# doing-science-to-stuff/ndt

Hardware: AMD Instinct MI355X
Metric: Mray/s (primary+shadow+reflect) at 1920x1080 (higher is better)
Workload: dtype f64

## Files before the change

### ndt_amd/csrc/ndt_device.hpp

```cpp
#pragma once
#include <hip/hip_runtime.h>
#include <stdint.h>

#define NDT_EPS   (1e-4)
#define NDT_EPS2  ((NDT_EPS) * (NDT_EPS))
#define NDT_INV_EPS2 (1.0 / (NDT_EPS2))
#define NDT_DBL_MAX 1.7976931348623157e308
#define NDT_PI 3.14159265358979323846

#define NDT_DEV __device__ __forceinline__

#define NDT_F_TYPE_MASK   0xff
#define NDT_F_GATE        0x100
#define NDT_F_INF_ENDS    0x200
#define NDT_F_USE_NORMALS 0x400
#define NDT_F_TRANSPARENT 0x800
#define NDT_F_BOX         0x1000
#define NDT_F_FACEBOX     0x2000
#define NDT_F_OBOX        0x4000
#define NDT_F_FACETREE    0x8000
#define NDT_F_FACEGROUPS  0x10000

enum { T_SPHERE = 0, T_HPLANE, T_HDISK, T_CYLINDER, T_HCYLINDER, T_ORTHOTOPE, T_HCUBE, T_HFACET, T_FACET };
enum { NDT_LIGHT_AMBIENT_ = 0, NDT_LIGHT_POINT_ = 1, NDT_LIGHT_DIRECTIONAL_ = 2, NDT_LIGHT_SPOT_ = 3 };
// ... 1211 lines not shown
            record_of(__ffsll((long long)any) - 1, flags, words, m, at, sph);
            const double t0 = word_of(lane, words, at, sph), t1 = word_of(lane + 64, words, at, sph);
            put(l_par, flags, words, m, t0, t1);
            cls_lds_sync();
        }
        while (any != 0ull) {
            const int k = __ffsll((long long)any) - 1;
            any &= any - 1ull;
            int n_flags = 0, n_words = 0, n_m = 0, n_at = 0, n_sph = 0;
            double t0 = 0.0, t1 = 0.0;
            if (any != 0ull) {
                record_of(__ffsll((long long)any) - 1, n_flags, n_words, n_m, n_at, n_sph);
                t0 = word_of(lane, n_words, n_at, n_sph);
                t1 = word_of(lane + 64, n_words, n_at, n_sph);
            }
            const long long rbits = __double_as_longlong(l_ref[k]);
            const int id = __builtin_amdgcn_readfirstlane((int)(rbits & 0xffffffffll));
            const int flags = __builtin_amdgcn_readfirstlane((int)(rbits >> 32));
            const double *rec = l_par + cur * par_stride;
            bool pass = open != 0 && ((want >> k) & 1ull);
            if ((flags & NDT_F_GATE) && pass) pass = bsphere_gate<N>(rec, sd_par, 0, o, v, min_dist);
            if (pass) {
                double res[N], nrm[N];
                if (isect<N, false>(rec, sd_par, 0, o, v, res, nrm)) {
                    const double dist = v_dist<N>(o, res);
                    if (dist > NDT_EPS && (dist + NDT_EPS < min_dist || min_dist < 0)) {
                        min_dist = dist;
                        best = id;
                    }
                    if (dist_limit == 0.0 || dist < dist_limit) {
                        open = 0;
                        last = id;
                    }
                }
            }
            cur ^= 1;
            if (any != 0ull) put(l_par + cur * par_stride, n_flags, n_words, n_m, t0, t1);
            cls_lds_sync();
            if (__ballot(open != 0) == 0ull) any = 0ull;
        }
        cls_lds_sync();
        NDT_STAMP(2);
        if (open) last = (int)(__double_as_longlong(l_ref[cnt - 1]) & 0xffffffffll);
        cls_lds_sync();
    }
}

#define NDT_KD_STACK 40
#define NDT_STACK_FLAG 0x40000000



struct KdStackLds {
    double *tu;
    int *node;
    int stride;
};

template <int N, int MW, bool LSTACK = false, bool UNI = false, bool LAZY_INV = false>
NDT_DEV void trace_kd(const double *blob, const SceneDesc &sd, VisitMask<MW> &mask, const double (&o)[N],
                      const double (&v)[N], double dist_limit, int &out_obj, int &out_prim
#ifdef NDT_PHASE_TIMING
                      , unsigned long long (&ph)[8], unsigned int (&cnt)[8], unsigned int (&occ)[8]
#endif
                      , KdStackLds ls = KdStackLds{}, ClsLds cl = ClsLds{}, const bool has_ray = true, double *box_slot = nullptr)
{
#ifdef NDT_PHASE_TIMING
    unsigned long long ph_last = __builtin_readcyclecounter();
#endif
#ifdef NDT_T1_KEEP_INV
    constexpr bool KEEP_INV = true;
#else
    constexpr bool KEEP_INV = (MW != 0);
#endif
    auto inv_of = [](double v_i) {
        double r;
        if (v_i < NDT_EPS2 && v_i >= 0.0)
            r = NDT_INV_EPS2;
        else if (v_i > -NDT_EPS2 && v_i <= 0.0)
            r = -NDT_INV_EPS2;
        else
            r = 1.0 / v_i;
        return r;
    };
    double v_inv[N];
    if (KEEP_INV && !LAZY_INV) {
#pragma unroll
        for (int i = 0; i < N; ++i) v_inv[i] = inv_of(v[i]);
    }
    auto inv_at = [&](int dim) {
        if constexpr (KEEP_INV) return v_pick<N>(v_inv, dim);
        else return inv_of(v_pick<N>(v, dim));
    };
    NDT_STAMP(5);

    double t_inf = NDT_DBL_MAX;
    int inf_obj = -1, inf_prim = -1;
    double lt = NDT_DBL_MAX;
    int l_obj = -1, l_prim = -1;

    int st_node[LSTACK ? 1 : NDT_KD_STACK];
    double st_a[LSTACK ? 1 : NDT_KD_STACK], st_tu[LSTACK ? 1 : NDT_KD_STACK];
    int sp = 0;
    int node = 0;
    double ntl = 0, ntu = 0;
    int st = 4;
    bool boxed = false;

    constexpr bool BITS = (MW == 1);
    unsigned long long cand = 0ull;
    int sec = 0, pos = 0, end = 0;
    double min_dist = -1;
    int best_obj = -1, best_prim = -1;
    int sub_i = 0, sub_end = 0, sub_owner = -1, sub_prim = -1;
    long long sub_live = -1;
    double sub_min = -1;

    if (!has_ray) {
        st = 3;
    } else if (sd.n_inf > 0) {
        st = 5;
        if (BITS) {
            cand = sd.inf_bits;
        } else {
            sec = sd.off_inf;
            pos = 0;
            end = sd.n_inf;
        }
    }

    while (true) {
        if (st == 4) {
            double tl = -NDT_DBL_MAX, tu = NDT_DBL_MAX;
            bool box = true;
#pragma unroll
            for (int i = 0; i < N; ++i) {
                if (box) {
                    double v_i = v[i], o_i = o[i];
                    if (!(fabs(v_i) < NDT_EPS2)) {
                        double tl_i = (blob[sd.off_bb + i] - o_i) / v_i;
                        double tu_i = (blob[sd.off_bb + N + i] - o_i) / v_i;
                        if (tl_i > tu_i) {
                            double tmp = tl_i;
                            tl_i = tu_i;
                            tu_i = tmp;
                        }
                        if (tl_i > tl) tl = tl_i;
                        if (tu_i < tu) tu = tu_i;
                        if (tu < -NDT_EPS) box = false;
                    }
                }
            }
            if (box) {
                tl -= NDT_EPS;
                tu += NDT_EPS;
                box = (tu >= -NDT_EPS) && (tl <= tu);
            }
            if (!box || sd.n_kd_nodes <= 0) {
                st = 3;
            } else {
                mask.clear(sd.mask_words);
                if (BITS && sd.gate_bits != 0ull) {
                    unsigned long long todo = sd.gate_bits, dead = 0ull;
                    while (todo != 0ull) {
                        const int id = __ffsll((long long)todo) - 1;
                        todo &= todo - 1ull;
                        const int b = sd.off_bs + id * (N + 2);
                        double c[N], oc[N];
                        blob_vec<N>(blob, b, c);
                        v_sub<N>(o, c, oc);
                        const double oc_len2 = v_dot<N>(oc, oc);
                        const double voc = v_dot<N>(v, oc);
                        const double voc2 = voc * voc;
                        const double desc = voc2 - oc_len2 + blob[b + N + 1];
                        if (desc < 0.0 || (voc > 0.0 && voc2 > desc)) dead |= 1ull << id;
                    }
                    mask.w[0] |= dead;
                }
                if (KEEP_INV && LAZY_INV) {
#pragma unroll
                    for (int i = 0; i < N; ++i) {
                        double v_i = v[i];
                        asm volatile("" : "+v"(v_i));
                        v_inv[i] = inv_of(v_i);
                    }
                }
                node = 0;
                ntl = tl;
                ntu = tu;
                st = 1;
            }
        }
        {
            while (st < 2) {
                NDT_OCC(0);
                if (st == 0) {
                    if (sp == 0) {
                        st = 3;
                    } else {
                        sp -= LSTACK ? ls.stride : 1;
                        double a;
                        if (LSTACK) {
                            const int parent = ls.node[sp];
                            ntu = ls.tu[sp];
                            const ndt_v2d prec = blob_pair(blob, sd.off_kd + 2 * parent);
                            const long long pw0 = __double_as_longlong(prec.x);
                            const int pdim = (int)(pw0 & 0xffffffffll);
                            const double pv_inv = inv_at(pdim);
                            a = (prec.y - v_pick<N>(o, pdim)) * pv_inv;
                            node = (pv_inv < NDT_EPS2) ? parent + 1 : (int)(pw0 >> 32);
                        } else {
                            node = st_node[sp];
                            a = st_a[sp];
                            ntu = st_tu[sp];
                        }
                        ntl = a - NDT_EPS;
                        st = ((lt > a) & !(ntu < 0.0)) ? 1 : 0;
                    }
                } else if (ntu < 0.0) {
                    st = 0;
                }
                if (st == 1) {
                    NDT_COUNT(0);
                    ndt_v2d rec = blob_pair(blob, sd.off_kd + 2 * node);
                    unsigned long long below = ~0ull;
                    if (BITS) {
                        double ns = blob[sd.off_nset + node];
#ifndef NDT_NO_T_HOIST
                        asm volatile("" : "+v"(rec.x), "+v"(rec.y), "+v"(ns));
#endif
                        below = (unsigned long long)__double_as_longlong(ns) & ~mask.w[0];
                    }
                    const long long w0 = __double_as_longlong(rec.x);
                    const int dim = (int)(w0 & 0xffffffffll);
                    if (BITS && below == 0ull) {
                        st = 0;
                    } else if (dim < 0) {
                        if (BITS) {
                            st = 2;
                            cand = below;
                        } else {
                            const long long w1 = __double_as_longlong(rec.y);
                            const int num = (int)(w1 >> 32);
                            st = num > 0 ? 2 : 0;
                            sec = sd.off_leaf;
                            pos = (int)(w1 & 0xffffffffll);
                            end = pos + num;
                        }
                    } else {
                        const double boundary = rec.y;
                        const double v_inv_i = inv_at(dim);
                        const double o_i = v_pick<N>(o, dim);
                        const bool swap = v_inv_i < NDT_EPS2;
                        const int left = node + 1, right = (int)(w0 >> 32);
                        const int near = swap ? right : left, far = swap ? left : right;
                        const double tp = (boundary - o_i) * v_inv_i;
                        const bool alive = lt > ntl;
                        const bool near_only = (ntu < tp - NDT_EPS) & alive;
                        const bool far_only = !near_only & (ntl > tp + NDT_EPS) & alive;
                        const bool both = !near_only & !far_only;
                        if (both & (lt > tp)) {
                            if (LSTACK) { ls.node[sp] = node; ls.tu[sp] = ntu; }
                            else { st_node[sp] = far; st_a[sp] = tp; st_tu[sp] = ntu; }
                            sp += LSTACK ? ls.stride : 1;
                        }
                        const bool go_near = near_only | (both & alive);
                        ntu = (both & alive) ? tp + NDT_EPS : ntu;
                        node = go_near ? near : far;
                        st = (go_near | far_only) ? 1 : 0;
                    }
                }
            }
        }
        NDT_STAMP(0);
        const bool have_list = st == 2 || st == 5, list_is_inf = st == 5;
        if (UNI ? (__ballot(have_list) == 0ull) : !have_list) break;

        min_dist = -1;
        best_obj = -1;
        best_prim = -1;
        bool list_open = have_list;
        bool scanned_together = false;
        if (UNI && MW == 0 && cl.base) {
            const bool elig = have_list && !list_is_inf && mask.hist_n >= 0;
            unsigned long long todo = __ballot(elig);
            const int n_listed = __popcll(__ballot(have_list));
            while (todo != 0ull) {
                const int leader = __ffsll((long long)todo) - 1;
                const int w0 = __builtin_amdgcn_readlane(sec + pos, leader), e0 = __builtin_amdgcn_readlane(sec + end, leader);
                bool mine = elig && sec + pos == w0;
                const unsigned long long group = __ballot(mine);
                todo &= ~group;
                if (__popcll(group) < cl.min_group && !(__popcll(group) == n_listed && n_listed >= 16)) mine = false;
                if (__ballot(mine) == 0ull) continue;
                double md;
                int best, last;
                NDT_STAMP(3);
#ifdef NDT_PHASE_TIMING
                cls_scan<N, MW>(blob, sd, mask, cl.base, mine, o, v, dist_limit, w0, e0, box_slot, boxed, md, best, last, ph, ph_last);
#else
                cls_scan<N, MW>(blob, sd, mask, cl.base, mine, o, v, dist_limit, w0, e0, box_slot, boxed, md, best, last);
#endif
                if (mine) {
                    min_dist = md;
                    best_obj = best;
                    best_prim = best;
                    mask.end_leaf(blob_int(blob, sd.off_kd + 2 * node, 1), last);
                    list_open = false;
                    scanned_together = true;
                }
            }
        }
        int gs = list_open ? 0 : 4;
        while (gs != 4) {
            int prim = -1;
// ... 218 lines not shown
```

### ndt_amd/csrc/ndt_kernels.hip

```cpp
#if NDT_DIMS <= 5 && !defined(NDT_OUTLINE_SMALL)
#define NDT_INLINE_LIBM 1
#endif
#if NDT_DIMS <= 7 && !defined(NDT_OUTLINE_SMALL)
#define NDT_SHADE_INLINE_ISECT 1
#endif
#include "ndt_kernels.hpp"
#include "ndt_shading.hpp"
#include <hip/hip_ext.h>
#include <stdlib.h>
#include <map>
#include <mutex>
#include <tuple>

#ifndef NDT_DIMS
#error "compile with -DNDT_DIMS=<3..10>"
#endif
#define NDT_CAT2(a, b) a##b
#define NDT_CAT(a, b) NDT_CAT2(a, b)

namespace NDT_CAT(ndt_d, NDT_DIMS) {

static constexpr int N = NDT_DIMS;


// ... 222 lines not shown
    mask.h0 = mask.h1 = mask.h2 = mask.h3 = 0u;
    mask.hist_n = -1;
    mask.slab_words = sd.mask_words;
    mask.ls.sets = nullptr;
    mask.ls.blob = gblob;
    mask.ls.words = sd.mask_words;
    mask.ls.off_lrange = sd.off_lrange;
    mask.ls.off_leaf = sd.off_leaf;
    mask.ls.cap = sd.hist_cap;
    if (MW == 0) {
        const long long lane_slot = (long long)blockIdx.x * blockDim.x + threadIdx.x;
        mask.ext = ws.mask_slab + lane_slot;
        mask.ext_stride = (int)ws.mask_slab_lanes;
        if (sd.off_lset > 0) mask.ls.sets = reinterpret_cast<const unsigned long long *>(gblob + sd.off_lset);
    }
}

NDT_DEV int seg_light_origin(const double *gblob, const SceneDesc &sd, int s)
{
    unsigned long long rest = ~sd.ambient_bits;
    for (int k = 0; k < s; ++k) rest &= rest - 1ull;
    const int li = __ffsll((long long)rest) - 1;
    const int w = sd.off_lights + li * (6 + 4 * N);
    const int type = blob_int(gblob, w, 0);
    return (type == NDT_LIGHT_POINT_ || type == NDT_LIGHT_SPOT_) ? w + 5 : -1;
}

typedef __attribute__((address_space(4))) const char *KernargBytes;
struct TraceKernargs {
    const double *gblob;
    SceneDesc sd;
    Workspace ws;
    TraceJob job;
};
constexpr size_t KARG_TRACE_WS = offsetof(TraceKernargs, ws);
constexpr size_t KARG_TRACE_JOB = offsetof(TraceKernargs, job);
#ifdef NDT_HEAD_STEPS
constexpr int trace_head_steps(int, int mw, bool, bool) { return mw != 0 ? (NDT_HEAD_STEPS) : 0; }
#else
constexpr int trace_head_steps(int n, int mw, bool lstack, bool prim)
{
    if (mw == 0) return 0;
    if (prim) return 7;
    if (n == 4 && mw == 4 && lstack) return 5;
    if (n == 4 && mw == 1 && !lstack) return 0;
    if (n == 5 && lstack) return 5;
    if (n == 6 && mw == 1 && !lstack) return 0;
    if (n == 8 && mw == 1 && !lstack) return 1;
    if (n == 10 && !lstack) return 5;
    if (n == 11 && !(mw == 1 && lstack)) return 0;
    return 7;
}
#endif
NDT_DEV KernargBytes karg_here()
{
    KernargBytes p = (KernargBytes)__builtin_amdgcn_kernarg_segment_ptr();
    asm volatile("" : "+s"(p));
    return p;
}
template <typename T> NDT_DEV T karg_get(KernargBytes p)
{
    static_assert(sizeof(T) % 4 == 0 && std::is_trivially_copyable<T>::value, "words");
    union { T v; unsigned int w[sizeof(T) / 4]; } u;
#pragma unroll
    for (size_t i = 0; i < sizeof(T) / 4; ++i) u.w[i] = reinterpret_cast<__attribute__((address_space(4))) const unsigned int *>(p)[i];
    return u.v;
}
#define NDT_KARG_PTR(obj, base, member) \
    (obj).member = *reinterpret_cast<__attribute__((address_space(4))) decltype((obj).member) const *>((base) + offsetof(decltype(obj), member))
NDT_DEV TracePart karg_trace_part(bool in_seg)
{
    const int at = in_seg ? (int)offsetof(TraceJob, seg) : (int)offsetof(TraceJob, dense);
    const KernargBytes kp = karg_here() + KARG_TRACE_JOB + __builtin_amdgcn_readfirstlane(at);
    TracePart p = karg_get<TracePart>(kp);
    NDT_KARG_PTR(p, kp, o); NDT_KARG_PTR(p, kp, v); NDT_KARG_PTR(p, kp, lim); NDT_KARG_PTR(p, kp, valid);
    NDT_KARG_PTR(p, kp, out_obj); NDT_KARG_PTR(p, kp, out_prim);
    return p;
}
NDT_DEV Workspace karg_trace_workspace(KernargBytes ka)
{
    const KernargBytes kp = ka + KARG_TRACE_WS;
    Workspace w = karg_get<Workspace>(kp);
    NDT_KARG_PTR(w, kp, ray_o); NDT_KARG_PTR(w, kp, ray_v); NDT_KARG_PTR(w, kp, frac); NDT_KARG_PTR(w, kp, depth_left);
    NDT_KARG_PTR(w, kp, hit_obj); NDT_KARG_PTR(w, kp, child_refl); NDT_KARG_PTR(w, kp, child_refr); NDT_KARG_PTR(w, kp, sh_mask);
    NDT_KARG_PTR(w, kp, count); NDT_KARG_PTR(w, kp, rng_key);
    return w;
}
NDT_DEV RenderGeom karg_trace_geom(KernargBytes ka)
{
    const KernargBytes kp = ka + KARG_TRACE_JOB + offsetof(TraceJob, rg);
    RenderGeom rg = karg_get<RenderGeom>(kp);
    NDT_KARG_PTR(rg, kp, samples); NDT_KARG_PTR(rg, kp, sample_keys);
    return rg;
}

#ifndef NDT_TICKET_AHEAD
#define NDT_TICKET_AHEAD 256
#endif
template <int MW, bool LDS, bool LSTACK = false, bool PRIM = false>
__global__ void __launch_bounds__(MW == 0 ? NDT_TRACE_T1_MAX_BLOCK : NDT_TRACE_MAX_BLOCK) k_trace(const double *__restrict__ gblob, SceneDesc sd, Workspace ws, TraceJob job)
{
    constexpr int STEPS = trace_head_steps(N, MW, LSTACK, PRIM);
    constexpr bool KARG = (STEPS & 1) != 0, SEG_ONCE = (STEPS & 2) != 0, LAZY = (STEPS & 4) != 0;
    extern __shared__ __attribute__((aligned(16))) double lds_blob[];
    const double *blob = gblob;
    if (LDS) {
        const int pairs = sd.trace_words >> 1;
        const ndt_v2d *src2 = reinterpret_cast<const ndt_v2d *>(gblob);
        ndt_v2d *dst2 = reinterpret_cast<ndt_v2d *>(lds_blob);
        int i = threadIdx.x;
        for (; i + 3 * (int)blockDim.x < pairs; i += 4 * blockDim.x) {
            const ndt_v2d a = src2[i], b = src2[i + blockDim.x], c = src2[i + 2 * blockDim.x], d = src2[i + 3 * blockDim.x];
            dst2[i] = a; dst2[i + blockDim.x] = b; dst2[i + 2 * blockDim.x] = c; dst2[i + 3 * blockDim.x] = d;
        }
        for (; i < pairs; i += blockDim.x) dst2[i] = src2[i];
        if ((sd.trace_words & 1) && threadIdx.x == 0) lds_blob[sd.trace_words - 1] = gblob[sd.trace_words - 1];
        __syncthreads();
        blob = lds_blob;
    }
    KdStackLds kstack{};
    if (LSTACK) {
        double *base = lds_blob + ((sd.trace_words + 1) & ~1);
        const int depth = sd.kd_depth + 1;
        kstack.stride = blockDim.x;
        kstack.tu = base + threadIdx.x;
        kstack.node = (int *)(base + (size_t)depth * blockDim.x) + threadIdx.x;
    }
    VisitMask<MW> mask;
    init_visit_mask<MW>(mask, gblob, sd, ws);
    ClsLds cls{};
    double *box_slot = nullptr;
    if (MW == 0 && !LDS) {
        const int wave = threadIdx.x >> 6, waves = blockDim.x >> 6;
        const int box_words = sd.off_obox > 0 ? N * 128 : 0;
        if (sd.off_obox > 0) box_slot = lds_blob + (size_t)wave * box_words + 2 * (threadIdx.x & 63);
        if (sd.cls_par_words > 0) {
            cls.base = lds_blob + (size_t)waves * box_words + (size_t)wave * cls_window_words<N>(sd.cls_par_words);
            cls.min_group = sd.cls_min_group;
        }
    }
    const int lane = __lane_id();
    const unsigned int probe_start = job.exit_log ? (unsigned int)wall_clock64() : 0u;
    unsigned int probe_batch = probe_start;
#ifdef NDT_PHASE_TIMING
    unsigned long long ph[8] = { 0, 0, 0, 0, 0, 0, 0, 0 };
    unsigned long long acc[24];
    for (int i = 0; i < 24; ++i) acc[i] = 0ull;
    unsigned long long out_last = __builtin_readcyclecounter();
    unsigned long long batch_mark = 0;
#endif
    const int bs = job.batch;
    const int sh = (bs == 64) ? 6 : (bs == 32) ? 5 : (bs == 16) ? 4 : 3;
    int seg_batches = 0, seg_batches_incl = 0, seg_cnt = 0;
    int seg_origin = -1;
    if (job.n_seg > 0) {
        seg_cnt = (lane < job.n_seg) ? job.seg_count[lane] : 0;
        const int excl = wave_excl_scan((seg_cnt + bs - 1) >> sh, seg_batches);
        seg_batches_incl = excl + ((seg_cnt + bs - 1) >> sh);
        if (SEG_ONCE && job.seg_light_origins && seg_cnt > 0) seg_origin = seg_light_origin(gblob, sd, lane);
    }
    long long dense_count = job.count, dense_begin = job.begin, seg_stride = job.seg_stride;
    if (job.levels) {
        const LevelRange cur = job.levels[job.seg_level];
        seg_stride = cur.seg_stride;
        LevelRange next;
        if (job.publish_level >= 0) {
            next.begin = cur.begin + cur.count;
            next.count = (long long)ws.counters[0] - next.begin;
            next.n_shadow = 0;
            if (next.count < 0 || (ws.counters[2] & 1) != 0) next.count = 0;
            next.seg_stride = (next.count + 63) & ~63LL;
            const bool sh_overflow = (long long)job.n_seg * next.seg_stride > ws.sh_cap;
            if (blockIdx.x == 0 && threadIdx.x < 64) {
                long long emitted = seg_cnt;
                for (int d = 32; d > 0; d >>= 1) emitted += __shfl_xor(emitted, d, 64);
                NDT_SEG_COUNTERS(ws, job.publish_level + 1)[lane] = 0;
                if (lane == 0) {
                    job_levels_mut(job)[job.publish_level].n_shadow = emitted;
                    LevelRange out = next;
                    if (sh_overflow) {
                        atomicOr(&ws.counters[2], 2);
                        const long long need = (long long)job.n_seg * next.seg_stride;
                        ws.counters[3] = need > 0x7fffffffLL ? 0x7fffffff : (int)need;
                        out.count = 0;
                        out.seg_stride = 0;
                    }
                    job_levels_mut(job)[job.publish_level + 1] = out;
                    ws.mail[job.publish_level + 1] = out;
                    __threadfence_system();
                    __hip_atomic_store(&ws.mail_tag[job.publish_level + 1], job.publish_tag, __ATOMIC_RELEASE, __HIP_MEMORY_SCOPE_SYSTEM);
                }
            }
            if (sh_overflow) next.count = 0;
        } else {
            next = job.levels[job.dense_level >= 0 ? job.dense_level : 0];
        }
        if (job.dense_level >= 0) {
            dense_begin = next.begin;
            dense_count = next.count;
// ... 66 lines not shown
            const int sb = (int)(b - dense_batches);
            const int s = __popcll(__ballot(lane < job.n_seg && seg_batches_incl <= sb));
            if (SEG_ONCE) origin_word = __builtin_amdgcn_readlane(seg_origin, __builtin_amdgcn_readfirstlane(s));
            else if (MW != 0 && job.seg_light_origins) origin_word = seg_light_origin(gblob, sd, __builtin_amdgcn_readfirstlane(s));
            const int first = (s > 0) ? __shfl(seg_batches_incl, s - 1, 64) : 0;
            const int cnt = __shfl(seg_cnt, s, 64);
            const int idx = (sb - first) * bs + lane;
            live = lane < bs && idx < cnt;
            g = (long long)s * seg_stride + (live ? idx : 0);
        } else {
            const long long r = b * bs + lane;
            live = lane < bs && r < dense_count;
            g = dense_begin + (live ? r : 0);
            if constexpr (KARG) {
                if (!PRIM && live) {
                    const int *valid = karg_trace_part(false).valid;
                    if (valid && valid[g] <= 0) live = false;
                }
            } else {
                if (!PRIM && live && job.dense.valid && job.dense.valid[g] <= 0) live = false;
            }
        }
        double o[N], v[N];
        const bool make = PRIM && !in_seg;
        if (PRIM && make && live) {
            if (KARG) {
                const KernargBytes ka = karg_here();
                live = primary_node<false, true>(gblob, sd, karg_trace_workspace(ka), karg_trace_geom(ka), g, o, v);
            } else {
                live = primary_node<false, true>(gblob, sd, ws, job.rg, g, o, v);
            }
        }
        if (live || MW == 0) {
        const TracePart part_here = KARG ? karg_trace_part(in_seg) : TracePart{};
        const TracePart &part = KARG ? part_here : in_seg ? job.seg : job.dense;
#ifdef NDT_TRACE_SKIP_KNOB
        if (job.skip_trace == 3) {
            for (int c = 0; c < N; ++c) { o[c] = (double)g; v[c] = 1.0; }
        } else
#endif
        if (live) {
            if (!make) {
                if (origin_word >= 0) blob_vec<N>(gblob, origin_word, o);
                else load_soa<N>(part.o, part.stride, g, o);
                load_soa<N>(part.v, part.stride, g, v);
            }
        } else {
#pragma unroll
            for (int c = 0; c < N; ++c) { o[c] = 0.0; v[c] = 0.0; }
        }
        const double lim = (live && part.lim) ? part.lim[g] : -1.0;
        int obj, prim;
#ifdef NDT_PHASE_TIMING
        unsigned int cnt[8] = { 0, 0, 0, 0, 0, 0, 0, 0 };
        unsigned int occ[8] = { 0, 0, 0, 0, 0, 0, 0, 0 };
        ph[6] += __builtin_readcyclecounter() - out_last;
        batch_mark = wall_clock64();
        if (job.skip_trace) {
            obj = (o[0] + v[0] + lim > 1e300) ? 0 : -1;
            prim = -1;
        } else
        trace_kd<N, MW, LSTACK, MW == 0, LAZY>(blob, sd, mask, o, v, lim, obj, prim, ph, cnt, occ, kstack, cls, live, box_slot);
        out_last = __builtin_readcyclecounter();
        if (ws.dbg && lane == __ffsll((long long)__ballot(1)) - 1) {
            const unsigned long long now = wall_clock64();
            atomicMax(&ws.dbg[40 + (int)in_seg], now - batch_mark);
            atomicAdd(&ws.dbg[42 + (int)in_seg], now - batch_mark);
            atomicAdd(&ws.dbg[44 + (int)in_seg], 1ull);
        }
        {
            const unsigned long long act = __ballot(1);
            if (lane == __ffsll((long long)act) - 1)
                for (int i = 0; i < 8; ++i) acc[(in_seg ? 16 : 8) + i] += occ[i];
            for (int i = 0; i < 6; ++i) acc[i] += cnt[i];
            acc[6] += 1ull;
            if (ws.dbg) {
                unsigned int nv = cnt[0], ng = cnt[1] + cnt[3], ni = cnt[2] + cnt[4];
                for (int d = 32; d > 0; d >>= 1) {
                    nv = max(nv, (unsigned int)__shfl_xor((int)nv, d, 64));
                    ng = max(ng, (unsigned int)__shfl_xor((int)ng, d, 64));
                    ni = max(ni, (unsigned int)__shfl_xor((int)ni, d, 64));
                }
                if (lane == __ffsll((long long)__ballot(1)) - 1) {
                    atomicMax(&ws.dbg[46], (unsigned long long)nv);
                    atomicMax(&ws.dbg[47], (unsigned long long)ng);
                    atomicMax(&ws.dbg[48], (unsigned long long)ni);
                    atomicMax(&ws.dbg[49], (unsigned long long)occ[0]);
                    atomicMax(&ws.dbg[50], (unsigned long long)occ[2]);
                    atomicMax(&ws.dbg[51], (unsigned long long)occ[4]);
                }
            }
        }
#else
#ifdef NDT_TRACE_SKIP_KNOB
        if (job.skip_trace) {
            obj = (o[0] + v[0] + lim > 1e300) ? 0 : -1;
            prim = -1;
        } else
#endif
        trace_kd<N, MW, LSTACK, MW == 0, LAZY>(blob, sd, mask, o, v, lim, obj, prim, kstack, cls, live, box_slot);
#endif
#ifdef NDT_TRACE_SKIP_KNOB
        if (job.skip_trace == 2 && obj == -1) live = false;
#endif
        if (live) {
            const TracePart out_here = KARG ? karg_trace_part(in_seg) : TracePart{};
            const TracePart &out = KARG ? out_here : part;
            out.out_obj[g] = obj;
            out.out_prim[g] = prim;
        }
        }
    }
    const unsigned int probe_left = job.exit_log ? (unsigned int)wall_clock64() : 0u;
    if (job.exit_log && lane == 0) {
        const unsigned int w = blockIdx.x * (blockDim.x / 64) + threadIdx.x / 64;
        if (8 * w + 7 < NDT_EXIT_LOG_WORDS) {
            job.exit_log[8 * w] = probe_start;
            job.exit_log[8 * w + 1] = probe_batch;
            job.exit_log[8 * w + 2] = (unsigned int)wall_clock64() | 1u;
            job.exit_log[8 * w + 3] = (__builtin_amdgcn_s_getreg((31 << 11) | 4) & 0xffffffu) | ((blockDim.x / 64) << 24);
            job.exit_log[8 * w + 4] = probe_left | 1u;
        }
    }
#ifdef NDT_PHASE_TIMING
    ph[6] += __builtin_readcyclecounter() - out_last;
    if (ws.dbg) {
        for (int i = 0; i < 24; ++i) {
            unsigned long long x = acc[i];
            for (int d = 32; d > 0; d >>= 1) x += __shfl_xor(x, d, 64);
            if (lane == 0 && x) atomicAdd(&ws.dbg[8 + i], x);
        }
        if (lane == 0) {
            for (int i = 0; i < 4; ++i) atomicAdd(&ws.dbg[i], ph[i]);
            atomicAdd(&ws.dbg[7], ph[7]);
            atomicAdd(&ws.dbg[32], ph[4]);
            atomicAdd(&ws.dbg[4], 1ull);
            atomicAdd(&ws.dbg[5], ph[5]);
            atomicAdd(&ws.dbg[6], ph[6]);
        }
    }
#endif
}

static_assert(std::is_same<decltype(&k_trace<1, true, true, false>), void (*)(const double *, SceneDesc, Workspace, TraceJob)>::value,
              "k_trace's parameters changed: change TraceKernargs with them");

#if defined(NDT_PHASE_TIMING) || defined(NDT_TRACE_SKIP_KNOB)
static int env_int(const char *name, int def)
{
    const char *e = getenv(name);
    return (e && *e) ? atoi(e) : def;
}
#else
static constexpr int env_int(const char *, int def) { return def; }
#endif

template <typename K> static int resident_blocks(K kernel, int block, size_t lds)
{
    static std::mutex mu;
    static std::map<std::tuple<int, const void *, int, size_t>, int> known;
    int dev = 0;
    (void)hipGetDevice(&dev);
    const auto key = std::make_tuple(dev, reinterpret_cast<const void *>(kernel), block, lds);
    std::lock_guard<std::mutex> lock(mu);
    auto it = known.find(key);
    if (it != known.end()) return it->second;
    int per_cu = 0;
    if (hipOccupancyMaxActiveBlocksPerMultiprocessor(&per_cu, kernel, block, lds) != hipSuccess || per_cu < 1) per_cu = 1;
    int cus = 256, v = 0;
    if (hipDeviceGetAttribute(&v, hipDeviceAttributeMultiprocessorCount, dev) == hipSuccess && v > 0) cus = v;
    known[key] = per_cu * cus;
    return per_cu * cus;
}

#define NDT_LAUNCH_TRACE(kernel, grid, block, lds)                                                             \
    do {                                                                                                       \
        if (ev_start)                                                                                          \
            hipExtLaunchKernelGGL((kernel), dim3((unsigned)(grid)), dim3(block), (std::uint32_t)(lds), s, ev_start, ev_stop, 0u, blob, sd, ws, job); \
        else                                                                                                   \
            hipLaunchKernelGGL((kernel), dim3((unsigned)(grid)), dim3(block), lds, s, blob, sd, ws, job);      \
    } while (0)
typedef void (*TraceKernel)(const double *, SceneDesc, Workspace, TraceJob);
static void launch_trace(hipStream_t s, const double *blob, SceneDesc sd, Workspace ws, TraceJob job, int tier,
// ... 658 lines not shown
```

### ndt_amd/csrc/ndt_probe.hip

```cpp
#include "ndt_ctx.hpp"

void ndt_impl::print_stream_probe(const unsigned int *wave_log, float km)
{
    std::vector<unsigned int> log((size_t)24 * NDT_STREAM_LOG_WAVES);
    if (hipMemcpy(log.data(), wave_log, log.size() * sizeof(unsigned int), hipMemcpyDeviceToHost) != hipSuccess) return;
    unsigned long long n[4] = { 0, 0, 0, 0 }, t[3] = { 0, 0, 0 }, parts[5] = { 0, 0, 0, 0, 0 };
    int waves = 0, busy_waves = 0;
    unsigned int t0 = 0, max_items = 0;
    bool any = false;
    for (int w = 0; w < NDT_STREAM_LOG_WAVES; ++w) {
        const unsigned int *q = &log[(size_t)24 * w];
        if (!q[9]) continue;
        if (!any || (int)(q[10] - t0) < 0) t0 = q[10];
        any = true;
    }
    double first_item = 1e30, last_item = 0, last_exit = 0, start_spread = 0;
    int hist[32] = { 0 };
    for (int w = 0; w < NDT_STREAM_LOG_WAVES; ++w) {
        const unsigned int *q = &log[(size_t)24 * w];
        if (!q[9]) continue;
        ++waves;
        const unsigned int items = q[0] + q[1] + q[2];
        if (items) ++busy_waves;
        if (items > max_items) max_items = items;
// ... 80 lines not shown
    double first = 1e30, last = 0, last_batch = 0, start_spread = 0;
    int simd_of_wave[16][4] = { { 0 } };
    int wpw = 12;
    for (int w = 0; w < NDT_EXIT_LOG_WORDS / 8; ++w)
        if (q[8 * w + 2]) {
            const double st_us = (q[8 * w] - t0) / 100.0, ex_us = (q[8 * w + 4] - t0) / 100.0;
            wpw = (int)(q[8 * w + 3] >> 24) > 0 && (q[8 * w + 3] >> 24) <= 16 ? (int)(q[8 * w + 3] >> 24) : wpw;
            ++simd_of_wave[w % wpw][(q[8 * w + 3] >> 4) & 3];
            if (st_us > start_spread) start_spread = st_us;
            if (ex_us < first) first = ex_us;
            if (ex_us > last) {
                last = ex_us;
                last_batch = (q[8 * w + 4] - q[8 * w + 1]) / 100.0;
            }
            const int bin = (int)(ex_us / 16.0);
            ++hist[bin > 63 ? 63 : bin];
        }
    std::string line;
    for (int bin = 0; bin < 64; ++bin)
        if (hist[bin]) {
            char buf[48];
            snprintf(buf, sizeof buf, " %d-%d:%d", bin * 16, bin * 16 + 16, hist[bin]);
            line += buf;
        }
    if (l == 0) {
        std::string m;
        for (int w = 0; w < wpw; ++w) {
            char buf[64];
            snprintf(buf, sizeof buf, " w%d:%d/%d/%d/%d", w, simd_of_wave[w][0], simd_of_wave[w][1], simd_of_wave[w][2], simd_of_wave[w][3]);
            m += buf;
        }
        fprintf(stderr, "ndt_hip: SIMD 0/1/2/3 of the workgroup's wavefronts (%d per workgroup):%s\n", wpw, m.c_str());
    }
    fprintf(stderr, "ndt_hip: trace launch %d: %d wavefronts start within %.1f us; first out of work at %.1f us, last at %.1f us (its last batch: %.1f us); exits per 16 us:%s\n",
            l, n_w, start_spread, first, last, last_batch, line.c_str());
}

void ndt_impl::print_exit_probe(const unsigned int *exit_log, int launches)
{
    std::vector<unsigned int> log((size_t)NDT_EXIT_LOG_LAUNCHES * NDT_EXIT_LOG_WORDS);
    if (hipMemcpy(log.data(), exit_log, log.size() * sizeof(unsigned int), hipMemcpyDeviceToHost) != hipSuccess) return;
    for (int l = 0; l < NDT_EXIT_LOG_LAUNCHES && l < launches; ++l) print_exit_probe_launch(log.data() + (size_t)l * NDT_EXIT_LOG_WORDS, l);
}

void ndt_impl::print_phase_timing(const unsigned long long *dbg)
{
    unsigned long long d[160];
    if (hipMemcpy(d, dbg, sizeof(d), hipMemcpyDeviceToHost) != hipSuccess || !d[4]) return;
    fprintf(stderr, "ndt_hip: wave cycles T %llu G %llu I %llu list-end %llu prologue %llu outside %llu over %llu waves\n", d[0], d[1], d[2], d[3], d[5], d[6], d[4]);
    if (d[7] || d[32])
        fprintf(stderr, "ndt_hip:    coherent leaf scan: fetching windows %llu, boxes / gates of the windows %llu (its intersections are in I)\n", d[32], d[7]);
    fprintf(stderr, "ndt_hip: per-ray counts over %llu rays: node visits %llu, face gates %llu (pass %llu), item gates %llu (pass %llu), isect hits %llu\n",
            d[14], d[8], d[9], d[10], d[11], d[12], d[13]);
    fprintf(stderr, "ndt_hip: batch time inside trace_kd (100 MHz wall clock): closest max %.1f us mean %.1f us, shadow max %.1f us mean %.1f us\n",
            d[40] / 100.0, d[44] ? d[42] / 100.0 / d[44] : 0.0, d[41] / 100.0, d[45] ? d[43] / 100.0 / d[45] : 0.0);
    fprintf(stderr, "ndt_hip: per-ray maxima: %llu node visits, %llu gates, %llu intersections; per-batch maxima: %llu T, %llu G, %llu I iterations\n",
            d[46], d[47], d[48], d[49], d[50], d[51]);
    if (d[58])
        fprintf(stderr, "ndt_hip: shade_emit per wavefront (wall-clock ticks, mean over %llu): load+isect %.0f, light tests %.0f, segment reserve %.0f, shadow stores %.0f, spawn %.0f; slowest wavefront %llu\n",
                d[58], (double)d[52] / d[58], (double)d[53] / d[58], (double)d[54] / d[58], (double)d[55] / d[58], (double)d[56] / d[58], d[59]);
    for (int kind = 0; kind < 2; ++kind) {
        const unsigned long long *q = d + 16 + 8 * kind;
        fprintf(stderr, "ndt_hip: loop occupancy (%s rays): T %.1f%% of %llu iters, G %.1f%% of %llu, I %.1f%% of %llu\n",
                kind ? "shadow" : "closest", q[0] ? 100.0 * q[1] / (64.0 * q[0]) : 0.0, q[0],
                q[2] ? 100.0 * q[3] / (64.0 * q[2]) : 0.0, q[2], q[4] ? 100.0 * q[5] / (64.0 * q[4]) : 0.0, q[4]);
        if (q[4])
            fprintf(stderr, "ndt_hip:    I iterations execute %.2f primitive types on average; the commonest type holds %.1f of %.1f active lanes\n",
                    (double)q[6] / q[4], (double)q[7] / q[4], (double)q[5] / q[4]);
    }
}
```

### ndt_amd/csrc/ndt_stream.hpp

```cpp

#include "ndt_finish.hpp"


#ifdef NDT_STREAM_PLAIN
NDT_DEV double cld(const double *p) { return *p; }
NDT_DEV void cst(double *p, double v) { *p = v; }
NDT_DEV int cldi(const int *p) { return *(const volatile int *)p; }
NDT_DEV void csti(int *p, int v) { *p = v; }
NDT_DEV unsigned long long cldu(const unsigned long long *p) { return *p; }
NDT_DEV void cstu(unsigned long long *p, unsigned long long v) { *p = v; }
#else
NDT_DEV double cld(const double *p)
{
    return __longlong_as_double((long long)__hip_atomic_load(reinterpret_cast<unsigned long long *>(const_cast<double *>(p)),
                                                             __ATOMIC_RELAXED, __HIP_MEMORY_SCOPE_AGENT));
}
NDT_DEV void cst(double *p, double v)
{
    __hip_atomic_store(reinterpret_cast<unsigned long long *>(p), (unsigned long long)__double_as_longlong(v), __ATOMIC_RELAXED,
                       __HIP_MEMORY_SCOPE_AGENT);
}
NDT_DEV int cldi(const int *p) { return __hip_atomic_load(const_cast<int *>(p), __ATOMIC_RELAXED, __HIP_MEMORY_SCOPE_AGENT); }
NDT_DEV void csti(int *p, int v) { __hip_atomic_store(p, v, __ATOMIC_RELAXED, __HIP_MEMORY_SCOPE_AGENT); }
NDT_DEV unsigned long long cldu(const unsigned long long *p)
// ... 410 lines not shown
    }
    {
        int t = 0, won = 0;
        if (lane < sa.n_seg) {
            t = cldi(&ctl->seg_tail[lane].v);
            if ((t & 63) != 0 && t < sa.seg_cap) won = atomicCAS(&ctl->seg_tail[lane].v, t, (t + 63) & ~63) == t;
        }
        unsigned long long winners = __ballot(won != 0);
        while (winners) {
            const int s = __ffsll((long long)winners) - 1;
            winners &= winners - 1;
            const int ts = __shfl(t, s, 64);
            const int pad = 64 - (ts & 63);
            if (lane < pad) csti(sa.sowner + (long long)s * sa.seg_cap + ts + lane, -1);
            drain();
            if (lane == 0) {
                const int bps = sa.seg_cap >> 6;
                const int old = atomicAdd(sa.sh_fill + s * bps + (ts >> 6), pad);
                if (old + pad == 64) ring_push(&ctl->sh_tail.v, sa.sh_ring, s * bps + (ts >> 6));
            }
        }
    }
}


#ifndef NDT_STREAM_MAX_BLOCK
#define NDT_STREAM_MAX_BLOCK 512
#endif
template <int MW, bool LDS, bool LSTACK = false>
__global__ void __launch_bounds__(NDT_STREAM_MAX_BLOCK) k_frame_stream(const double *gblob, SceneDesc sd, Workspace ws, RenderGeom rg,
                                                                      StreamArgs sa)
{
    extern __shared__ __attribute__((aligned(16))) double lds_blob[];
    const double *blob = gblob;
    if (LDS) {
        const int pairs = sd.trace_words >> 1;
        const ndt_v2d *src2 = reinterpret_cast<const ndt_v2d *>(gblob);
        ndt_v2d *dst2 = reinterpret_cast<ndt_v2d *>(lds_blob);
        int i = threadIdx.x;
        for (; i + 3 * (int)blockDim.x < pairs; i += 4 * blockDim.x) {
            const ndt_v2d a = src2[i], b = src2[i + blockDim.x], c = src2[i + 2 * blockDim.x], d = src2[i + 3 * blockDim.x];
            dst2[i] = a; dst2[i + blockDim.x] = b; dst2[i + 2 * blockDim.x] = c; dst2[i + 3 * blockDim.x] = d;
        }
        for (; i < pairs; i += blockDim.x) dst2[i] = src2[i];
        if ((sd.trace_words & 1) && threadIdx.x == 0) lds_blob[sd.trace_words - 1] = gblob[sd.trace_words - 1];
        __syncthreads();
        blob = lds_blob;
    }
    KdStackLds kstack{};
    if (LSTACK) {
        double *base = lds_blob + ((sd.trace_words + 1) & ~1);
        const int depth = sd.kd_depth + 1;
        kstack.stride = blockDim.x;
        kstack.tu = base + threadIdx.x;
        kstack.node = (int *)(base + (size_t)depth * blockDim.x) + threadIdx.x;
    }
    VisitMask<MW> mask;
    init_visit_mask<MW>(mask, gblob, sd, ws);
    double *box_slot = nullptr;
    if (MW == 0 && !LDS && sd.off_obox > 0) box_slot = lds_blob + (size_t)(threadIdx.x >> 6) * (N * 128) + 2 * (threadIdx.x & 63);
    __shared__ int wg_over;
    if (threadIdx.x == 0) wg_over = 0;
    __syncthreads();
    const bool watcher = threadIdx.x < 64;
    StreamCtl *ctl = sa.ctl;
    const int lane = __lane_id();
    const int n_prim_batches = sa.n_primary >> 6;
    const int home = blockIdx.x % NDT_PRIM_SHARDS;
    int shard = home;
    unsigned shards_alive = (1u << NDT_PRIM_SHARDS) - 1u;
    const unsigned long long t_begin = wall_clock64();
    int idle_rounds = 0;
    int tk_sec = -1, tk_sec_shard = home;
    int tk_sh = -1, tk_fin = -1;
    unsigned int pr_n[4] = { 0, 0, 0, 0 }, pr_t[4] = { 0, 0, 0, 0 }, pr_first = 0, pr_last = 0;
    unsigned int pr_pop = 0, pr_load = 0, pr_trace = 0;
    unsigned int pr_trace_sh = 0, pr_up = 0;
    unsigned long long pr_mark = 0, pr_top = 0;
    WaveStats stats = { 0, 0, 0, 0ull };
    int items = 0;
    int light_next = -1;
    while (true) {
        if ((items++ & 15) == 15 && cldi(&ctl->abort.v) != 0) break;
        if (sa.wave_log) pr_top = wall_clock64();
        int kind = 0, id = -1;
        if (light_next >= 0) {
            kind = 3;
            id = light_next;
            light_next = -1;
        } else if (sec_pop(sa, home, false, tk_sec, tk_sec_shard, id)) {
            kind = 1;
        } else {
            while (shards_alive != 0u && kind == 0) {
                if ((shards_alive >> shard) & 1u) {
                    int k = 0;
                    if (lane == 0) k = atomicAdd(&ctl->prim_head[shard].v, 1);
                    k = __shfl(k, 0, 64);
                    const int b = k * NDT_PRIM_SHARDS + shard;
                    if (b < n_prim_batches) {
                        kind = 1;
                        id = (sa.root_begin >> 6) + b;
                    } else {
                        shards_alive &= ~(1u << shard);
                    }
                }
                if (kind == 0) shard = (shard + 1) % NDT_PRIM_SHARDS;
            }
            if (kind == 0) {
                if (ring_pop(&ctl->sh_head.v, sa.sh_ring, tk_sh, id)) kind = 2;
                else if (ring_pop(&ctl->fin_head.v, sa.fin_ring, tk_fin, id)) kind = 3;
                else if ((watcher || (idle_rounds & 3) == 3) && sec_pop(sa, home, true, tk_sec, tk_sec_shard, id))
                    kind = 1;
            }
        }
        if (sa.wave_log && kind != 0) {
            pr_mark = wall_clock64();
            if (pr_first == 0) pr_first = (unsigned int)(pr_mark - t_begin) | 1u;
            pr_pop += (unsigned int)(pr_mark - pr_top);
        }
        int up_node = 0;
        bool up_active = false;
        int parts_done = 0;
        if (kind == 1 || kind == 2) {
            idle_rounds = 0;
            const bool is_shadow = kind == 2;
            long long slot;
            if (is_shadow) {
                const int bps = sa.seg_cap >> 6;
                const int s = id / bps, k = id - s * bps;
                slot = (long long)s * sa.seg_cap + (long long)k * 64 + lane;
            } else {
                slot = (long long)id * 64 + lane;
            }
            const bool make = sa.fused != 0 && !is_shadow && slot < sa.root_begin + sa.n_primary;
            double o[N], v[N];
            int tag;
            if (make) tag = primary_node<true>(gblob, sd, ws, rg, slot, o, v) ? rg.max_depth : 0;
            else tag = is_shadow ? cldi(sa.sowner + slot) : cldi(ws.depth_left + slot);
            const bool valid = is_shadow ? tag >= 0
                                         : tag > 0 && (slot >= sa.root_begin + sa.n_primary || (slot >= sa.valid_begin && slot < sa.valid_end));
            double lim = -1.0;
            int obj = -1, prim = -1;
            if (valid) {
                if (!make) {
                    cload_soa<N>(is_shadow ? ws.so : ws.ray_o, slot, o);
                    cload_soa<N>(is_shadow ? ws.sv : ws.ray_v, slot, v);
                }
                if (is_shadow) lim = cld(ws.slim + slot);
                unsigned long long pr_a = 0;
                if (sa.wave_log) {
                    asm volatile("s_waitcnt vmcnt(0)" ::: "memory");
                    pr_a = wall_clock64();
                    pr_load += (unsigned int)(pr_a - pr_mark);
                }
#ifdef NDT_PHASE_TIMING
                {
                    unsigned long long ph[8] = {};
                    unsigned int cnt[8] = {}, occ[8] = {};
                    trace_kd<N, MW, LSTACK>(blob, sd, mask, o, v, lim, obj, prim, ph, cnt, occ, kstack, ClsLds{}, true, box_slot);
                }
#else
                trace_kd<N, MW, LSTACK>(blob, sd, mask, o, v, lim, obj, prim, kstack, ClsLds{}, true, box_slot);
#endif
                if (sa.wave_log) {
                    const unsigned int dt = (unsigned int)(wall_clock64() - pr_a);
                    pr_trace += dt;
                    if (is_shadow) pr_trace_sh += dt;
                }
            } else {
#pragma unroll
                for (int c = 0; c < N; ++c) { o[c] = 0.0; v[c] = 0.0; }
            }
            if (is_shadow) {
                if (valid) {
                    csti(ws.sobj + slot, obj);
                    csti(ws.sprim + slot, prim);
                }
                drain();
                const int nb = tag >> 6;
                const int nb_prev = __shfl_up(nb, 1, 64);
                const bool valid_prev = __shfl_up((int)valid, 1, 64) != 0;
                const bool head = valid && (lane == 0 || !valid_prev || nb_prev != nb);
                const unsigned long long heads = __ballot(head), valids = __ballot(valid);
                if (head) {
                    const unsigned long long above = (lane < 63) ? (heads >> (lane + 1)) << (lane + 1) : 0ull;
                    const int end = above ? __ffsll((long long)above) - 1 : 64;
                    const unsigned long long span = (end < 64 ? (1ull << end) - 1ull : ~0ull) & ~((1ull << lane) - 1ull);
                    const int run = __popcll(valids & span);
                    const int old = atomicSub(sa.sh_pending + nb, run);
                    if (old == run) ring_push(&ctl->fin_tail.v, sa.fin_ring, nb);
                }
            } else {
                bool light_now, any_shaded, final_root;
                stream_shade_batch(blob, gblob, sd, ws, rg, sa, id, valid, tag, o, v, obj, prim, stats, home, up_node, up_active, light_now,
                                   any_shaded, final_root);
                if (sa.fused && final_root) stats.ref += finish_pixel<true>(gblob, sd, ws, rg, N, slot, sa.rgba, sa.depth_out);
                parts_done = any_shaded ? 1 : 2;
                if (light_now) light_next = id;
            }
        } else if (kind == 3) {
            idle_rounds = 0;
            up_active = stream_light_batch(blob, gblob, sd, ws, rg, sa, id);
            up_node = id * 64 + lane;
            parts_done = 1;
        }
        if (kind == 1 || kind == 3) {
            unsigned long long pr_b = 0;
            if (sa.wave_log) pr_b = wall_clock64();
            complete_up(gblob, sd, ws, sa, rg, up_node, up_active, stats);
            if (sa.wave_log) pr_up += (unsigned int)(wall_clock64() - pr_b);
            if (lane == 0) atomicSub(&ctl->outstanding[id % NDT_PRIM_SHARDS].v, 64 * parts_done);
// ... 109 lines not shown
```

Measured before the change: 4513.

## Store far child and split distance on LDS kd stack; test leaf sets at leaves

```diff
diff --git a/ndt_amd/csrc/ndt_device.hpp b/ndt_amd/csrc/ndt_device.hpp
--- a/ndt_amd/csrc/ndt_device.hpp
+++ b/ndt_amd/csrc/ndt_device.hpp
@@ -1287,16 +1287,16 @@
 
 
 struct KdStackLds {
-    double *tu;
+    double *t;
     int *node;
     int stride;
 };
 
-template <int N, int MW, bool LSTACK = false, bool UNI = false, bool LAZY_INV = false>
+template <int N, int MW, bool LSTACK = false, bool UNI = false, bool LAZY_INV = false, bool POP = false, bool LEAF_SETS = false>
 NDT_DEV void trace_kd(const double *blob, const SceneDesc &sd, VisitMask<MW> &mask, const double (&o)[N],
                       const double (&v)[N], double dist_limit, int &out_obj, int &out_prim
 #ifdef NDT_PHASE_TIMING
-                      , unsigned long long (&ph)[8], unsigned int (&cnt)[8], unsigned int (&occ)[8]
+                      , unsigned long long (&ph)[8], unsigned int (&cnt)[12], unsigned int (&occ)[8]
 #endif
                       , KdStackLds ls = KdStackLds{}, ClsLds cl = ClsLds{}, const bool has_ray = true, double *box_slot = nullptr)
 {
@@ -1336,6 +1336,7 @@
 
     int st_node[LSTACK ? 1 : NDT_KD_STACK];
     double st_a[LSTACK ? 1 : NDT_KD_STACK], st_tu[LSTACK ? 1 : NDT_KD_STACK];
+    static_assert(LSTACK || !POP, "POP is a layout of the LDS stack");
     int sp = 0;
     int node = 0;
     double ntl = 0, ntu = 0;
@@ -1423,6 +1424,7 @@
                 node = 0;
                 ntl = tl;
                 ntu = tu;
+                if (POP) ls.t[-ls.stride] = tu;
                 st = 1;
             }
         }
@@ -1434,10 +1436,19 @@
                         st = 3;
                     } else {
                         sp -= LSTACK ? ls.stride : 1;
+                        NDT_COUNT(6);
+#ifdef NDT_PHASE_TIMING
+                        cnt[8] += (__lane_id() == __ffsll((long long)__ballot(1)) - 1);
+#endif
                         double a;
-                        if (LSTACK) {
+                        if (POP) {
+                            node = ls.node[sp];
+                            a = ls.t[sp];
+                            const double below = ls.t[sp - ls.stride];
+                            ntu = sp == 0 ? below : below + NDT_EPS;
+                        } else if (LSTACK) {
                             const int parent = ls.node[sp];
-                            ntu = ls.tu[sp];
+                            ntu = ls.t[sp];
                             const ndt_v2d prec = blob_pair(blob, sd.off_kd + 2 * parent);
                             const long long pw0 = __double_as_longlong(prec.x);
                             const int pdim = (int)(pw0 & 0xffffffffll);
@@ -1451,6 +1462,9 @@
                         }
                         ntl = a - NDT_EPS;
                         st = ((lt > a) & !(ntu < 0.0)) ? 1 : 0;
+#ifdef NDT_PHASE_TIMING
+                        cnt[7] += (st == 0);
+#endif
                     }
                 } else if (ntu < 0.0) {
                     st = 0;
@@ -1459,7 +1473,8 @@
                     NDT_COUNT(0);
                     ndt_v2d rec = blob_pair(blob, sd.off_kd + 2 * node);
                     unsigned long long below = ~0ull;
-                    if (BITS) {
+                    constexpr bool SETS_AT_LEAVES = BITS && LEAF_SETS;
+                    if (BITS && !SETS_AT_LEAVES) {
                         double ns = blob[sd.off_nset + node];
 #ifndef NDT_NO_T_HOIST
                         asm volatile("" : "+v"(rec.x), "+v"(rec.y), "+v"(ns));
@@ -1472,7 +1487,8 @@
                         st = 0;
                     } else if (dim < 0) {
                         if (BITS) {
-                            st = 2;
+                            if (SETS_AT_LEAVES) below = (unsigned long long)__double_as_longlong(blob[sd.off_nset + node]) & ~mask.w[0];
+                            st = (SETS_AT_LEAVES && below == 0ull) ? 0 : 2;
                             cand = below;
                         } else {
                             const long long w1 = __double_as_longlong(rec.y);
@@ -1494,8 +1510,9 @@
                         const bool near_only = (ntu < tp - NDT_EPS) & alive;
                         const bool far_only = !near_only & (ntl > tp + NDT_EPS) & alive;
                         const bool both = !near_only & !far_only;
-                        if (both & (lt > tp)) {
-                            if (LSTACK) { ls.node[sp] = node; ls.tu[sp] = ntu; }
+                        if (POP ? (both & alive) : (both & (lt > tp))) {
+                            if (POP) { ls.node[sp] = far; ls.t[sp] = tp; }
+                            else if (LSTACK) { ls.node[sp] = node; ls.t[sp] = ntu; }
                             else { st_node[sp] = far; st_a[sp] = tp; st_tu[sp] = ntu; }
                             sp += LSTACK ? ls.stride : 1;
                         }
diff --git a/ndt_amd/csrc/ndt_kernels.hip b/ndt_amd/csrc/ndt_kernels.hip
--- a/ndt_amd/csrc/ndt_kernels.hip
+++ b/ndt_amd/csrc/ndt_kernels.hip
@@ -298,6 +298,29 @@
     return 7;
 }
 #endif
+constexpr int trace_walk_mask(int mw, bool lstack) { return (lstack ? 1 : 0) | (mw == 1 ? 2 : 0); }
+#ifdef NDT_POP_STEP
+constexpr int trace_walk_steps(int, int mw, bool lstack, bool) { return (NDT_POP_STEP) & trace_walk_mask(mw, lstack); }
+#else
+constexpr int trace_walk_steps(int n, int mw, bool lstack, bool prim)
+{
+    constexpr int take[10][6] = {
+        { 3, 3, 1, 1, 2, 2 },
+        { 3, 3, 0, 1, 2, 2 },
+        { 2, 2, 1, 0, 2, 2 },
+        { 3, 2, 0, 0, 0, 2 },
+        { 0, 0, 0, 1, 2, 2 },
+        { 3, 0, 1, 0, 2, 2 },
+        { 2, 2, 0, 1, 2, 2 },
+        { 3, 2, 0, 0, 2, 2 },
+        { 2, 2, 0, 1, 2, 2 },
+        { 2, 2, 0, 0, 2, 2 },
+    };
+    const int col = lstack ? (mw == 1 ? 0 : 2) + (prim ? 1 : 0) : 4 + (prim ? 1 : 0);
+    if (n < 3 || n > 12 || (mw != 1 && !(mw == 4 && lstack))) return 0;
+    return take[n - 3][col] & trace_walk_mask(mw, lstack);
+}
+#endif
 NDT_DEV KernargBytes karg_here()
 {
     KernargBytes p = (KernargBytes)__builtin_amdgcn_kernarg_segment_ptr();
@@ -348,6 +371,8 @@
 {
     constexpr int STEPS = trace_head_steps(N, MW, LSTACK, PRIM);
     constexpr bool KARG = (STEPS & 1) != 0, SEG_ONCE = (STEPS & 2) != 0, LAZY = (STEPS & 4) != 0;
+    constexpr int WALK = trace_walk_steps(N, MW, LSTACK, PRIM);
+    constexpr bool POP = (WALK & 1) != 0, LEAF_SETS = (WALK & 2) != 0;
     extern __shared__ __attribute__((aligned(16))) double lds_blob[];
     const double *blob = gblob;
     if (LDS) {
@@ -369,7 +394,7 @@
         double *base = lds_blob + ((sd.trace_words + 1) & ~1);
         const int depth = sd.kd_depth + 1;
         kstack.stride = blockDim.x;
-        kstack.tu = base + threadIdx.x;
+        kstack.t = base + threadIdx.x + (POP ? blockDim.x : 0);
         kstack.node = (int *)(base + (size_t)depth * blockDim.x) + threadIdx.x;
     }
     VisitMask<MW> mask;
@@ -391,6 +416,7 @@
 #ifdef NDT_PHASE_TIMING
     unsigned long long ph[8] = { 0, 0, 0, 0, 0, 0, 0, 0 };
     unsigned long long acc[24];
+    unsigned long long pops[3] = { 0, 0, 0 };
     for (int i = 0; i < 24; ++i) acc[i] = 0ull;
     unsigned long long out_last = __builtin_readcyclecounter();
     unsigned long long batch_mark = 0;
@@ -563,7 +589,7 @@
         const double lim = (live && part.lim) ? part.lim[g] : -1.0;
         int obj, prim;
 #ifdef NDT_PHASE_TIMING
-        unsigned int cnt[8] = { 0, 0, 0, 0, 0, 0, 0, 0 };
+        unsigned int cnt[12] = { 0, 0, 0, 0, 0, 0, 0, 0, 0, 0, 0, 0 };
         unsigned int occ[8] = { 0, 0, 0, 0, 0, 0, 0, 0 };
         ph[6] += __builtin_readcyclecounter() - out_last;
         batch_mark = wall_clock64();
@@ -571,7 +597,7 @@
             obj = (o[0] + v[0] + lim > 1e300) ? 0 : -1;
             prim = -1;
         } else
-        trace_kd<N, MW, LSTACK, MW == 0, LAZY>(blob, sd, mask, o, v, lim, obj, prim, ph, cnt, occ, kstack, cls, live, box_slot);
+        trace_kd<N, MW, LSTACK, MW == 0, LAZY, POP, LEAF_SETS>(blob, sd, mask, o, v, lim, obj, prim, ph, cnt, occ, kstack, cls, live, box_slot);
         out_last = __builtin_readcyclecounter();
         if (ws.dbg && lane == __ffsll((long long)__ballot(1)) - 1) {
             const unsigned long long now = wall_clock64();
@@ -585,6 +611,7 @@
                 for (int i = 0; i < 8; ++i) acc[(in_seg ? 16 : 8) + i] += occ[i];
             for (int i = 0; i < 6; ++i) acc[i] += cnt[i];
             acc[6] += 1ull;
+            for (int i = 0; i < 3; ++i) pops[i] += cnt[6 + i];
             if (ws.dbg) {
                 unsigned int nv = cnt[0], ng = cnt[1] + cnt[3], ni = cnt[2] + cnt[4];
                 for (int d = 32; d > 0; d >>= 1) {
@@ -609,7 +636,7 @@
             prim = -1;
         } else
 #endif
-        trace_kd<N, MW, LSTACK, MW == 0, LAZY>(blob, sd, mask, o, v, lim, obj, prim, kstack, cls, live, box_slot);
+        trace_kd<N, MW, LSTACK, MW == 0, LAZY, POP, LEAF_SETS>(blob, sd, mask, o, v, lim, obj, prim, kstack, cls, live, box_slot);
 #endif
 #ifdef NDT_TRACE_SKIP_KNOB
         if (job.skip_trace == 2 && obj == -1) live = false;
@@ -640,6 +667,11 @@
             unsigned long long x = acc[i];
             for (int d = 32; d > 0; d >>= 1) x += __shfl_xor(x, d, 64);
             if (lane == 0 && x) atomicAdd(&ws.dbg[8 + i], x);
+        }
+        for (int i = 0; i < 3; ++i) {
+            unsigned long long x = pops[i];
+            for (int d = 32; d > 0; d >>= 1) x += __shfl_xor(x, d, 64);
+            if (lane == 0 && x) atomicAdd(&ws.dbg[60 + i], x);
         }
         if (lane == 0) {
             for (int i = 0; i < 4; ++i) atomicAdd(&ws.dbg[i], ph[i]);
diff --git a/ndt_amd/csrc/ndt_probe.hip b/ndt_amd/csrc/ndt_probe.hip
--- a/ndt_amd/csrc/ndt_probe.hip
+++ b/ndt_amd/csrc/ndt_probe.hip
@@ -156,6 +156,9 @@
         fprintf(stderr, "ndt_hip:    coherent leaf scan: fetching windows %llu, boxes / gates of the windows %llu (its intersections are in I)\n", d[32], d[7]);
     fprintf(stderr, "ndt_hip: per-ray counts over %llu rays: node visits %llu, face gates %llu (pass %llu), item gates %llu (pass %llu), isect hits %llu\n",
             d[14], d[8], d[9], d[10], d[11], d[12], d[13]);
+    if (d[60])
+        fprintf(stderr, "ndt_hip: traversal stack over %llu rays: pops %llu, of them dropped at once %llu; T iterations with a pop in them %llu (of %llu)\n",
+                d[14], d[60], d[61], d[62], d[16] + d[24]);
     fprintf(stderr, "ndt_hip: batch time inside trace_kd (100 MHz wall clock): closest max %.1f us mean %.1f us, shadow max %.1f us mean %.1f us\n",
             d[40] / 100.0, d[44] ? d[42] / 100.0 / d[44] : 0.0, d[41] / 100.0, d[45] ? d[43] / 100.0 / d[45] : 0.0);
     fprintf(stderr, "ndt_hip: per-ray maxima: %llu node visits, %llu gates, %llu intersections; per-batch maxima: %llu T, %llu G, %llu I iterations\n",
diff --git a/ndt_amd/csrc/ndt_stream.hpp b/ndt_amd/csrc/ndt_stream.hpp
--- a/ndt_amd/csrc/ndt_stream.hpp
+++ b/ndt_amd/csrc/ndt_stream.hpp
@@ -486,7 +486,7 @@
         double *base = lds_blob + ((sd.trace_words + 1) & ~1);
         const int depth = sd.kd_depth + 1;
         kstack.stride = blockDim.x;
-        kstack.tu = base + threadIdx.x;
+        kstack.t = base + threadIdx.x;
         kstack.node = (int *)(base + (size_t)depth * blockDim.x) + threadIdx.x;
     }
     VisitMask<MW> mask;
@@ -590,7 +590,7 @@
 #ifdef NDT_PHASE_TIMING
                 {
                     unsigned long long ph[8] = {};
-                    unsigned int cnt[8] = {}, occ[8] = {};
+                    unsigned int cnt[12] = {}, occ[8] = {};
                     trace_kd<N, MW, LSTACK>(blob, sd, mask, o, v, lim, obj, prim, ph, cnt, occ, kstack, ClsLds{}, true, box_slot);
                 }
 #else
```

New measurement: 4588, median of 6. +1.7%, better.
